# k2kobayashi/crank

Hardware: AMD Instinct MI355X
Metric: train frames/sec (higher is better)
Workload: dtype bf16; 1 GPU; vqvae trainer step (all sub-updates), VCC2020-shaped synthetic 80-dim mlfb, 64 utterances x 500 frames per GPU, 14 speakers; trainer=vqvae, global_batch=64, batch_len=500, parallelism=dp1

## Files before the change

### crank_amd/_lib.py

```python
import ctypes
import os
from .config import cfg
from ctypes import c_char_p, c_double, c_float, c_int, c_longlong, c_ulonglong, c_void_p

_HERE = os.path.dirname(os.path.abspath(__file__))
LIB_PATH = cfg.lib_path or os.path.join(_HERE, "libcrank_hip.so")
_lib = None

ERRORS = {1: "invalid argument", 2: "HIP runtime error", 3: "unsupported shape/configuration"}


class NetDesc(ctypes.Structure):
    _fields_ = [
        ("kind", c_int), ("in_ch", c_int), ("out_ch", c_int), ("kernel_size", c_int), ("layers", c_int),
        ("stacks", c_int), ("res_ch", c_int), ("gate_ch", c_int), ("skip_ch", c_int), ("aux_ch", c_int),
        ("conv_ch", c_int), ("causal", c_int), ("use_bias", c_int), ("slope", c_float), ("dropout", c_float),
    ]


COLLATE_MAX_STREAMS = 8


class CollateStream(ctypes.Structure):
    _fields_ = [("src", c_void_p), ("ld", c_int), ("col0", c_int), ("ncols", c_int), ("dst", c_void_p)]
# ... 8 lines not shown
    ]


P, I, LL, ULL, F, D = c_void_p, c_int, c_longlong, c_ulonglong, c_float, c_double

SIGNATURES = {
    "crk_net_create": (P, [ctypes.POINTER(NetDesc)]),
    "crk_net_destroy": (None, [P]),
    "crk_net_param_count": (LL, [P]),
    "crk_net_conv_count": (I, [P]),
    "crk_net_conv_info": (I, [P, I, ctypes.POINTER(c_longlong)]),
    "crk_net_saved_bytes": (LL, [P, I, I]),
    "crk_net_reserve": (I, [P, I, I]),
    "crk_net_scratch_bytes": (LL, [P, I, I]),
    "crk_debug_alloc_count": (LL, []),
    "crk_debug_net_paths": (I, [P, I, I]),
    "crk_seed_next": (I, [P, P, P]),
    "crk_nets_wnorm_bwd": (I, [I, P, P]),
    "crk_nets_prepare": (I, [I, P, P, ULL, P, P]),
    "crk_net_forward": (I, [P, P, ULL, P, I, P, I, P, I, P, I, I, I, ULL, P]),
    "crk_net_backward": (I, [P, P, ULL, P, P, I, P, I, P, I, P, I, F, P, I, P, I, I, I, ULL, P]),
    "crk_net_backward_scaled": (I, [P, P, ULL, P, P, I, P, I, P, I, P, I, F, P, I, P, I, I, I, ULL, P, P, P]),
    "crk_net_embed_grad_supported": (I, [P, I, I, I]),
    "crk_net_backward_embed": (I, [P, P, ULL, P, P, I, P, I, P, I, P, I, F, P, I, I, I, ULL, P, LL, I, I, I, P, P]),
    "crk_vq_forward": (I, [P, I, P, I, I, I, P, P, I, P, I, P]),
    "crk_vq_forward_fused": (I, [P, I, P, I, P, I, P, I, I, I, P, P, I, P, I, P, P, P, P, P]),
    "crk_vq_image_bytes": (LL, [I, I]),
    "crk_vq_image_build_multi": (I, [I, P, P, I, P, P]),
    "crk_vq_ema_scratch_bytes": (LL, [I, I, I]),
    "crk_vq_ema_stats": (I, [P, I, P, I, I, I, P, P, P, P]),
    "crk_vq_ema_apply": (I, [P, P, P, P, P, I, I, D, D, P]),
    "crk_vq_ema_partial": (I, [P, I, P, I, I, I, P, P]),
    "crk_vq_ema_reduce_multi": (I, [I, P, P, P, P, P, P, P]),
    "crk_vq_ema_apply_multi": (I, [I, P, P, P, P, P, P, P, D, D, P]),
    "crk_vq_ema_partial_multi": (I, [I, P, P, P, P, P, P, P, P]),
    "crk_vq_ema_reduce_size_multi": (I, [I, P, P, P, P, P, P, P, D, D, P]),
    "crk_vq_ema_blend_multi": (I, [I, P, P, P, P, P, P, D, P]),
    "crk_vq_ema_blend_image_multi": (I, [I, P, P, P, P, P, P, D, P, P]),
    "crk_stft_loss_multi_fwd": (I, [P, I, P, I, I, I, I, I, P, P, P, P, F, P, P, P]),
    "crk_stft_loss_multi_fwd_grad": (I, [P, I, P, I, I, I, I, I, P, P, P, P, F, P, P, I, P, P]),
    "crk_stft_loss_multi_bwd": (I, [P, I, P, I, I, I, I, I, P, P, P, P, F, P, P, I, P]),
    "crk_loss_scratch_floats": (I, []),
    "crk_masked_loss_fwd": (I, [P, I, P, I, F, P, LL, I, I, P, P, P]),
    "crk_masked_loss_bwd": (I, [P, I, P, I, F, P, LL, I, I, P, P, P, I, P, I, P]),
    "crk_masked_loss_both_fwd": (I, [P, I, P, I, P, LL, I, P, P, P]),
    "crk_weighted_sum": (I, [I, P, P, F, P, P]),
# ... 123 lines not shown
```

### crank_amd/config.py

```python
import contextlib
import os
import types

_get = os.environ.get


def _flag(name, default):
    v = _get(name)
    return default if v is None else v not in ("0", "")


def _read():
    return types.SimpleNamespace(
        precision=_get("CRANK_AMD_PRECISION", "bf16"),
        lib_path=_get("CRANK_AMD_LIB") or None,
        default_yaml=_get("CRANK_DEFAULT_YAML") or None,
        overlap_c=int(_get("CRANK_AMD_OVERLAP_C", "1") or 0),
        separate_ce=_flag("CRANK_AMD_SEPARATE_CE", False),
        separate_commit=_flag("CRANK_AMD_SEPARATE_COMMIT", False),
        recon_dense=_flag("CRANK_AMD_RECON_DENSE", False),
        stft_two_pass=_flag("CRANK_AMD_STFT_TWO_PASS", False),
        cond_sums=_flag("CRANK_AMD_COND_SUMS", True),
        force_dist=_flag("CRANK_AMD_FORCE_DIST", False),
        dist_backend=_get("CRANK_AMD_DIST_BACKEND") or None,
        dp_graph_collectives=_flag("CRANK_AMD_DP_GRAPH_COLLECTIVES", True),
        capture_mode=_get("CRANK_AMD_CAPTURE_MODE", "thread_local"),
        test_refuse_capture_rank=_get("CRANK_AMD_TEST_REFUSE_CAPTURE_RANK"),
    )


cfg = _read()


def reload():
    cfg.__dict__.update(_read().__dict__)


def torchrun():
    r = _get("RANK")
    return (None if r is None else int(r)), int(_get("LOCAL_RANK", "0")), int(_get("WORLD_SIZE", "1"))


@contextlib.contextmanager
def override(**kw):
    unknown = [k for k in kw if not hasattr(cfg, k)]
# ... 9 lines not shown
```

### crank_amd/csrc/conv_kernels.h

```cpp
#pragma once
#include <vector>

#include "common.h"
#include "switches.h"

#define CRK_TM 128

enum { MODE_PLAIN = 0, MODE_RESFWD = 1, MODE_BWDA = 2 };

struct ConvP {
  const float* xa; int lda; int cinA; float scaleA;
  const float* xb; int ldb; int cinB; float scaleB;
  int act_in; float slope;
  float drop_p; unsigned long long drop_seed;
  const unsigned long long* drop_seed_ptr;
  int cin, cin_pad;
  const float* xc; int ldc; int cinC; int cinC_pad;
  const uint16_t* w_hi; const uint16_t* w_lo;
  const uint16_t* wc_hi; const uint16_t* wc_lo;
  const uint16_t* w2_hi; const uint16_t* w2_lo;
  const float* bias; const float* bias2a; const float* bias2b;
  int cout, cout_pad, ktaps, dil, off0;
  int B, T, tiles_per_utt;
  float* y; int ldy; int accumulate; int act_out; float out_scale;
// ... 27 lines not shown

struct ConvEntry {
  int cout, cin, k;
  long long off_g, off_v, off_b;
  long long fw_off; int fw_rows, fw_kp, fw_row0;
  long long bw_off; int bw_rows, bw_kp, bw_col0;
  long long pt_off; int pt_rows, pt_row0, pt_cx, pt_taps, pt_tap0; float pt_scale;
  int pt_groups;
  long long pb_off;
  long long norm_off;
  long long fr_off; int fr_mode;
  long long bfr_off; int bfr_mode;
};

struct StackLayer {
  long long f_conv, f_aux, f_os;
  long long w_conv, w_aux, w_os;
  long long b_conv, b_out, b_skip;
  int dil, off0;
};
struct StackP {
  const float* x0;
  const float* c; int ldc; int aux_ch, aux_pad;
  float* saved;
  uint16_t *xb_hi, *xb_lo;
  uint16_t *zb_hi, *zb_lo;
  uint16_t *tb_hi, *tb_lo, *sg_hi, *sg_lo;
  uint16_t *cb_hi, *cb_lo;
  float* skip;
  const float* params;
  const uint16_t* whi; const uint16_t* wlo;
  const StackLayer* layers;
  int B, T, L, ktaps;
  int hl, hr, max_off;
  int tmo, tiles_per_utt;
  float drop_p; unsigned long long drop_seed; const unsigned long long* drop_seed_ptr;
  int o_xlo, o_zhi, o_zlo, o_chi, o_clo, o_whi, o_wlo, o_bias, o_tab, w_bytes, lds_bytes;
  int nw;
  int dbg;
  int ft, fh;
  int ft1;
  int o_zs, o_cs;
  int o_xf;
  const float* x_in; int ldx_in, in_ch, kp_first;
  long long f_first, b_first;
  long long f_h1, b_h1, f_h2, b_h2;
// ... 156 lines not shown
```

### crank_amd/csrc/net.hip

```cpp
#include <math.h>
#include <stdlib.h>
#include <string.h>

#include <deque>
#include <vector>

#include "conv_kernels.h"

struct crk_net_desc {
  int kind;
  int in_ch, out_ch, kernel_size, layers, stacks;
  int res_ch, gate_ch, skip_ch, aux_ch;
  int conv_ch;
  int causal;
  int use_bias;
  float slope;
  float dropout;
};

enum { ROLE_FIRST = 0, ROLE_CONV = 1, ROLE_AUX = 2, ROLE_OUT = 3, ROLE_SKIP = 4, ROLE_LAST1 = 5, ROLE_LAST2 = 6, ROLE_PLAIN = 7 };

struct ConvMeta {
  int role, layer, dilation;
};
// ... 620 lines not shown

static void tag_forward(Net* n, const float* saved, int B, int T, const Call& k, bool x3f) {
  if (!saved || !k.keep) return;
  const Net::FwdTag tag = {saved, B, T, k.mode, x3f};
  for (int i = 0; i < n->fwd_tag_count; i++)
    if (n->fwd_tags[i].saved == saved) { n->fwd_tags[i] = tag; return; }
  n->fwd_tags[n->fwd_tag_next] = tag;
  n->fwd_tag_next = (n->fwd_tag_next + 1) % 32;
  if (n->fwd_tag_count < 32) n->fwd_tag_count++;
}
static int check_forward_tag(const Net* n, const float* saved, int B, int T, int flags, int want, bool expects_x3f) {
  for (int i = 0; i < n->fwd_tag_count; i++) {
    const Net::FwdTag& t = n->fwd_tags[i];
    if (t.saved != saved) continue;
    if (t.B == B && t.T == T && t.mode == want && (want != 2 || t.x3f == expects_x3f)) return CRK_OK;
    fprintf(stderr, "[crank_hip] crk_net_backward: flags 0x%x (plane layout %d%s, B %d, T %d) do not match the forward that wrote this "
                    "workspace (layout %d%s, B %d, T %d): CRK_FLAG_PRECISE pairs with CRK_FLAG_PRECISE, CRK_FLAG_PRECISE | CRK_FLAG_BWD_PLAIN "
                    "with CRK_FLAG_FWD_PRECISE, plain with plain\n", flags, want, expects_x3f ? " x3f" : "", B, T, t.mode, t.x3f ? " x3f" : "", t.B, t.T);
    return CRK_ERR_ARG;
  }
  return CRK_OK;
}

struct FwdIo {
  const float* params; const float* x; int ldx; const float* c; int ldc; float* y; int ldy; float* saved; int B, T; hipStream_t s;
};
enum { FWD_CHAIN, FWD_CHAIN_LAYERS, FWD_FOLDED, FWD_FUSED, FWD_LAYERS };
static int fwd_form(const Net* n, const Route& rt, const Call& k, bool x3f, int* form) {
  if (n->d.kind == 2) { *form = rt.fused ? FWD_CHAIN : FWD_CHAIN_LAYERS; return CRK_OK; }
  const bool io16 = k.in16 && k.out16;
  if ((x3f || rt.gen_split) && !io16) {
    fprintf(stderr, "[crank_hip] crk_net_forward: x / y must be 16-byte aligned with row strides that are multiples of 4 floats\n");
    return CRK_ERR_ARG;
  }
  if (x3f || (rt.fold_fwd && io16)) *form = FWD_FOLDED;
  else if (rt.gen_split) return CRK_ERR_UNSUPPORTED;
  else *form = rt.fused ? FWD_FUSED : FWD_LAYERS;
  return CRK_OK;
}

static int fwd_chain(const Net* n, const Shape* r, const Call& k, const FwdIo& a) {
  if (!a.saved && k.keep) return CRK_ERR_ARG;
  const Route& rt = r->route[k.precise];
  const PsTables& Tb = r->ps;
  const long long N = (long long)a.B * a.T;
  PsP p = ps_base(n, a.B, a.T, a.params);
  p.x = a.x; p.ldx = a.ldx; p.cin = n->d.in_ch; p.y = a.y; p.ldy = a.ldy;
  if (k.keep) {
// ... 12 lines not shown
  const crk_net_desc& d = n->d;
  const int L = n->L;
  const long long N = (long long)a.B * a.T;
  if (L > 1 && !a.saved) return CRK_ERR_ARG;
  const float* in = a.x; int ldin = a.ldx;
  for (int i = 0; i < L; i++) {
    const ConvEntry& e = n->ents[n->idx_plain[i]];
    const int dil = n->meta[n->idx_plain[i]].dilation;
    const bool last = i == L - 1;
    ConvP p = conv_fw(n, a.B, a.T, e, a.params, in, ldin, last ? a.y : a.saved + (long long)i * N * d.conv_ch, last ? a.ldy : d.conv_ch);
    p.act_in = (i == 0) ? ACT_NONE : ACT_LRELU;
    p.ktaps = e.k; p.dil = dil; p.off0 = -((e.k - 1) / 2) * dil;
    RUN(conv_go(p, MODE_PLAIN, k.precise, a.s));
    in = p.y; ldin = p.ldy;
  }
  return CRK_OK;
}
static StackP stack_fwd_params(const Net* n, const Call& k, const FwdIo& a, bool lo) {
  const long long N = (long long)a.B * a.T;
  const GatedB16 gf = gated_b16(n, N);
  uint16_t* b16 = reinterpret_cast<uint16_t*>(a.saved + saved_f32_floats(n, N));
  StackP sp = stack_fwd_shape(n, a.B, a.T);
  sp.c = a.c; sp.ldc = a.ldc; sp.params = a.params;
  sp.skip = a.saved + gated_f32(n, N).skip;
  sp.whi = n->whi; sp.wlo = n->wlo; sp.layers = n->d_layers;
  if (!k.keep) return sp;
  sp.saved = a.saved;
  sp.xb_hi = b16 + gf.xb_hi; sp.zb_hi = b16 + gf.zb_hi; sp.tb_hi = b16 + gf.tb_hi; sp.sg_hi = b16 + gf.sg_hi;
  if (n->d.aux_ch > 0) sp.cb_hi = b16 + gf.cb_hi;
  if (!lo) { sp.fin_hi = b16 + gf.f_hi; sp.head_hi = b16 + gf.head_hi; return sp; }
  sp.xb_lo = b16 + gf.xb_lo; sp.zb_lo = b16 + gf.zb_lo; sp.tb_lo = b16 + gf.tb_lo; sp.sg_lo = b16 + gf.sg_lo;
  if (n->d.aux_ch > 0) sp.cb_lo = b16 + gf.cb_lo;
  return sp;
}
static int fwd_folded(const Net* n, const Route& rt, const Call& k, const FwdIo& a, bool x3f) {
  const crk_net_desc& d = n->d;
  const ConvEntry& ef = n->ents[n->idx_first];
  const ConvEntry& e1 = n->ents[n->idx_last1];
  const ConvEntry& e2 = n->ents[n->idx_last2];
  StackP sp = stack_fwd_params(n, k, a, false);
  sp.x_in = a.x; sp.ldx_in = a.ldx; sp.in_ch = d.in_ch; sp.kp_first = ef.fw_kp;
  sp.f_first = ef.fr_off; sp.b_first = ef.off_b;
  sp.f_h1 = e1.fr_off; sp.b_h1 = e1.off_b; sp.f_h2 = e2.fr_off; sp.b_h2 = e2.off_b;
  sp.y = a.y; sp.ldy = a.ldy; sp.out_ch = d.out_ch; sp.head_scale = (float)sqrt(1.0 / n->L);
  if (x3f || rt.gen_split) sp.ts_stride = ts_plane_stride((long long)a.B * a.T);
  if (x3f) { RUN(stack2x_fwd_plan(sp)); return launch_stack2x_fwd(sp, a.s); }
// ... 43 lines not shown
    const int dil = n->meta[n->idx_conv[l]].dilation;
    ConvP p = conv_fw(n, a.B, a.T, ec, a.params, X + l * P, 64, (l < L - 1) ? X + (l + 1) * P : nullptr, 64);
    p.ktaps = ec.k; p.dil = dil; p.off0 = fwd_off0(n, ec.k, dil);
    if (d.dropout > 0.f) { p.drop_p = d.dropout; p.drop_seed = layer_seed(k.seed_val, l); p.drop_seed_ptr = k.seed_ptr; }
    if (d.aux_ch > 0) {
      const ConvEntry& ea = n->ents[n->idx_aux[l]];
      p.xc = a.c; p.ldc = a.ldc; p.cinC = ea.cin; p.cinC_pad = ea.fw_kp;
      p.wc_hi = n->whi + ea.fw_off; p.wc_lo = n->wlo + ea.fw_off;
    }
    p.w2_hi = n->whi + eo.fw_off; p.w2_lo = n->wlo + eo.fw_off;
    p.bias2a = eo.off_b >= 0 ? a.params + eo.off_b : nullptr;
    p.bias2b = es.off_b >= 0 ? a.params + es.off_b : nullptr;
    p.skip = SKIP; p.skip_init = (l == 0);
    p.sv_ta = a.saved + lay.ta + l * P; p.sv_sb = a.saved + lay.sb + l * P; p.sv_z = a.saved + lay.z + l * P;
    RUN(conv_go(p, MODE_RESFWD, k.precise, a.s));
  }
  ConvP h1 = conv_fw(n, a.B, a.T, n->ents[n->idx_last1], a.params, SKIP, 64, H1, 64);
  h1.scaleA = (float)sqrt(1.0 / L); h1.act_in = head_act;
  RUN(conv_go(h1, MODE_PLAIN, k.precise, a.s));
  ConvP h2 = conv_fw(n, a.B, a.T, n->ents[n->idx_last2], a.params, H1, 64, a.y, a.ldy);
  h2.act_in = head_act;
  return conv_go(h2, MODE_PLAIN, k.precise, a.s);
}
extern "C" int crk_net_forward(void* h, const float* params, unsigned long long version, const float* x, int ldx,
                               const float* c, int ldc, float* y, int ldy, float* saved, int B, int T, int flags,
                               unsigned long long seed, void* stream) {
  Net* n = (Net*)h;
  if (!n || !params || !x || !y || B <= 0 || T <= 0) return CRK_ERR_ARG;
  const FwdIo a = {.params = params, .x = x, .ldx = ldx, .c = c, .ldc = ldc, .y = y, .ldy = ldy, .saved = saved, .B = B, .T = T,
                   .s = (hipStream_t)stream};
  const Call k = call_facts(flags, seed, true, x, ldx, y, ldy, nullptr, nullptr);
  const Shape* r = find_shape(n, B, T);
  if (!r) return not_reserved("crk_net_forward");
  const Route& rt = r->route[k.precise];
  const bool x3f = k.mode == 2 && r->route[0].x3f;
  RUN(ensure_prepared(n, params, version, a.s));
  tag_forward(n, saved, B, T, k, x3f);
  if (n->d.kind != 2 && (!saved || (n->d.aux_ch > 0 && !c))) return CRK_ERR_ARG;
  int form;
  RUN(fwd_form(n, rt, k, x3f, &form));
  switch (form) {
    case FWD_CHAIN: return fwd_chain(n, r, k, a);
    case FWD_CHAIN_LAYERS: return fwd_chain_layers(n, k, a);
    case FWD_FOLDED: return fwd_folded(n, rt, k, a, x3f);
    case FWD_FUSED: return fwd_fused(n, r, k, a);
  }
  return fwd_layers(n, k, a);
}

static int stack_cpg(const Net* n, int B, int T) {
  const int ncpu = (T + 63) / 64;
  const int groups = crk_sw().wg_groups;
  const int gsz = (B + groups - 1) / groups;
  int cpg = gsz * ncpu;
  if (crk_sw().wg_fill && n->d.kind != 2 && n->L > 0 && 256 / n->L > groups) {
    const int fill = 256 / n->L;
    const int c = (B * ncpu + fill - 1) / fill;
    if (c >= 1 && c < cpg) cpg = c;
  }
  return cpg < 1 ? 1 : cpg;
}
static int stack_groups(const Net* n, int B, int T) {
  const int total = B * ((T + 63) / 64), cpg = stack_cpg(n, B, T);
  return (total + cpg - 1) / cpg;
}

static int usum_nseg(const Net* n, int B, int T) {
  const int ncpu = (T + 63) / 64;
  return (stack_cpg(n, B, T) + 2 * ncpu - 2) / ncpu;
}
// ... 562 lines not shown
```

### crank_amd/csrc/stack2_kernels.hip

```cpp
#include "conv_kernels.h"

#include "stack_common.h"

#define S2_NCU 256
#define S2_PAIR_FACTOR 1.0

#if defined(S2_ABL) && (S2_ABL & 2)
#define mfma_bf16(a, b, c) s2_fake_mfma(a, b, c)
__device__ __forceinline__ f32x16 s2_fake_mfma(bf16x8 a, bf16x8 b, f32x16 c) {
  asm volatile("" ::"v"(a), "v"(b));
  return c;
}
#endif
#if defined(S2_ABL) && (S2_ABL & 4)
#define lds_frag(p) s2_fake_frag(p)
__device__ __forceinline__ bf16x8 s2_fake_frag(const unsigned char* p) {
  const unsigned v = (unsigned)(size_t)p;
  const sk_u32x4 q = {v, v, v, v};
  return __builtin_bit_cast(bf16x8, q);
}
#endif
#ifdef S2_PROF
__device__ unsigned long long s2_prof_buf[256 * 8 * 16];
__device__ unsigned long long s2_prof_res[1024 * 4];
// ... 62 lines not shown
  if (FOLD) {
    const __amdgpu_buffer_rsrc_t rxi = sk_rsrc(p.x_in, (long)p.B * p.T * p.ldx_in);
    int xrow = xr0, xcol = xc0;
#pragma unroll
    for (int u = 0; u < XQ; u++) {
      const int c4 = xcol * 4, t = t0 - p.hl + xrow;
      const bool on = xrow < R && t >= 0 && t < p.T && c4 < p.in_ch;
      xq[u] = __builtin_amdgcn_raw_buffer_load_b128(rxi, on ? (int)(((nbase + t) * p.ldx_in + c4) * 4) : SK_OOB, 0, 0);
      xrow += xdr; xcol += xdc;
      if (xcol >= ppr) { xcol -= ppr; xrow++; }
    }
    if (res_wave) {
      const int KF = p.kp_first >> 4;
#pragma unroll
      for (int kc = 0; kc < 8; kc++) awf[kc] = S2_WLOAD(p.f_first + (mt * KF + (kc < KF ? kc : 0)) * 512);
    }
#pragma unroll
    for (int q = 0; q < 4; q++)
      bfq[q] = (res_wave && p.b_first >= 0) ? *reinterpret_cast<const sk_f32x4*>(p.params + p.b_first + 32 * mt + 8 * q + 4 * half) : sk_f32x4{0.f, 0.f, 0.f, 0.f};
  }
  constexpr int CNQ = R * 16, CPER = AKC > 0 ? (CNQ + NT - 1) / NT : 1;
  float av[CPER][4];
  if (AKC > 0) {
#pragma unroll
    for (int it = 0; it < CPER; it++) {
      const int idx = tid + it * NT, r = idx >> 4, c4 = (idx & 15) << 2;
      const int tt = t0 - p.hl + r;
      const bool on = idx < CNQ && tt >= 0 && tt < p.T;
      const long n = nbase + tt;
#pragma unroll
      for (int j = 0; j < 4; j++) av[it][j] = (on && c4 + j < p.aux_ch) ? p.c[n * p.ldc + c4 + j] : 0.f;
    }
  }
  S2_T(12)
  constexpr int NBI = 16 * 256 / NT;
  float bv[NBI];
#pragma unroll
  for (int k = 0; k < NBI; k++) {
    const int i0 = __builtin_amdgcn_readfirstlane(tid + k * NT) & ~63;
    const int l = i0 >> 8, c0 = i0 & 255, c = c0 + lane;
    bv[k] = 0.f;
    if (l < p.L) {
      const long long bo = c0 < 128 ? p.layers[l].b_conv : (c0 < 192 ? p.layers[l].b_out : p.layers[l].b_skip);
      if (bo >= 0) bv[k] = p.params[bo + (c0 < 128 ? c : (c0 < 192 ? c - 128 : c - 192))] * ((c0 >= 128 && c0 < 192) ? 0.70710678118654752440f : 1.f);
    }
  }
  int tabv[2] = {0, 0};
#pragma unroll
  for (int u = 0; u < 2; u++)
    if (tid + u * NT < p.L * (int)(sizeof(StackLayer) / 4)) tabv[u] = reinterpret_cast<const int*>(p.layers)[tid + u * NT];
  static_assert(16 * sizeof(StackLayer) / 4 <= 2 * NT, "two table words per thread");

  constexpr int NWB = KT == 3 ? 3 : 4, NWB1 = KT == 3 ? 3 : 2;
  sk_u32x4 wa[NWB][4];
// ... 543 lines not shown
```

### crank_amd/net/module/vqvae2.py

```python
import torch

from ... import ops, parallel
from .flat import FlatModel
from .mlfb import LogMelFilterBankLayer
from .pwg import KIND_GENERATOR, MAX_CHANNELS, HipStack


class Quantizer:

    def __init__(self, owner, prefix, emb_dim, emb_size, decay=0.99, eps=1e-5, ema_flag=False, bdt_flag=False):
        self.owner, self.prefix = owner, prefix
        self.emb_dim, self.emb_size = emb_dim, emb_size
        self.decay, self.eps, self.ema_flag, self.bdt_flag = decay, eps, ema_flag, bdt_flag
        self.cb_offset = None
        self.training = True
        self.bucket, self.slot = None, 0
        self._img, self._img_epoch = None, -1

    def entries(self, base):
        self.cb_offset = base
        return [(self.prefix + "embedding.weight", base, (self.emb_size, self.emb_dim))]

    @property
    def n_params(self):
# ... 267 lines not shown
        if todo:
            ops.vq_image_build([q.weight for q in todo], [q._img for q in todo])
            for q in todo:
                q._img_epoch = self.codebook_epoch

    def train(self, mode=True):
        super().train(mode)
        for q in self.quantizers:
            q.training = mode
        return self

    @property
    def spkr_table(self):
        o = self.emb_offset
        return self.flat.data[o: o + self.spkr_size * self.emb_size].view(self.spkr_size, self.emb_size)

    def spkr_embedding(self, h):
        return ops.concat_embed(None, None, self.spkr_table, h, self, self.emb_offset, self.flat)

    def _get_dec_h(self, dec_h, spkrvec):
        a, b = dec_h if isinstance(dec_h, (tuple, list)) else (dec_h, None)
        if spkrvec is not None:
            if torch.is_grad_enabled() and ops.embed_owned_ok(self.decoders[0].net, a, b, spkrvec):
                return ops.concat_embed_owned(a, b, self.spkr_table, spkrvec, self, self.emb_offset)
            return ops.concat_embed(a, b, self.spkr_table, spkrvec, self, self.emb_offset, self.flat)
        return dec_h if b is None else torch.cat([a, b], dim=-1)

    def _pre(self, x):
        return self.preprocess_layer(x) if self.conf["use_raw"] else x

    def encode(self, x, enc_h=None):
        out = []
        cur = x
        dims = self.conf["emb_dim"][: self.conf["n_vq_stacks"]]
        ebuf = torch.empty(x.shape[0], x.shape[1], sum(dims), device=x.device, dtype=torch.float32)
        col = 0
        for n in range(self.conf["n_vq_stacks"]):
            cur = self.encoders[n](cur, c=enc_h if n == 0 else None, out=(ebuf, col))
            col += dims[n]
            out.append(cur)
        return out

    def decode(self, enc, dec_h, use_ema=True, detach=False, need_decoded=True, commit_mask=None, want_commit=False):
        dec = None
        emb_idxs, qxs, qidxs = [], [], []
        self._commits = []
        self.refresh_images()
# ... 95 lines not shown
```

### crank_amd/ops.py

```python
import ctypes

import torch

from . import _lib
from .config import cfg
from ._lib import check, ptr, stream_ptr

_PRECISION = cfg.precision


def set_precision(name):
    global _PRECISION
    if name not in ("bf16", "bf16x3", "bf16x3f"):
        raise ValueError(f"unknown precision {name!r} (bf16 | bf16x3 | bf16x3f)")
    _PRECISION = name


def get_precision():
    return _PRECISION


CRK_FLAG_PRECISE = 1
CRK_FLAG_NO_PARAM_GRAD = 2
CRK_FLAG_NO_SAVE = 4
CRK_FLAG_DEFER_WNORM = 8
CRK_FLAG_SEED_ON_DEVICE = 16
CRK_FLAG_FWD_PRECISE = 32
CRK_FLAG_BWD_PLAIN = 64


def _flags(skip_param_grads=False, no_save=False, precision=None, defer_wnorm=False, backward=False):
    prec = precision or _PRECISION
    if prec == "bf16x3f":
        pbits = CRK_FLAG_FWD_PRECISE if backward else (CRK_FLAG_PRECISE | CRK_FLAG_BWD_PLAIN)
    else:
        pbits = CRK_FLAG_PRECISE if prec == "bf16x3" else 0
    return (pbits | (CRK_FLAG_NO_PARAM_GRAD if skip_param_grads else 0) | (CRK_FLAG_NO_SAVE if no_save else 0)
            | (CRK_FLAG_DEFER_WNORM if defer_wnorm else 0))


class _ScalarArena:

    def __init__(self, device, n=256):
        self.buf = torch.empty(n, device=device, dtype=torch.float32)
        self.pos = 0


_ARENA = None


def begin_scalar_arena(device):
# ... 60 lines not shown
        self.seed_state.fill_(v)

    def next_seed(self):
        out = torch.empty(1, dtype=torch.int64, device=self.seed_state.device)
        check(_lib.lib().crk_seed_next(ptr(self.seed_state), ptr(out), stream_ptr()), "crk_seed_next")
        return out

    def saved_bytes(self, B, T):
        key = (B, T, _PRECISION)
        v = self._saved_bytes.get(key)
        if v is None:
            check(_lib.lib().crk_net_reserve(self.handle, B, T), "crk_net_reserve")
            v = self._saved_bytes[key] = _lib.lib().crk_net_saved_bytes(self.handle, B, T)
        return v

    def embed_grad_supported(self, B, T):
        key = ("embed", B, T, _PRECISION)
        v = self._saved_bytes.get(key)
        if v is None:
            self.saved_bytes(B, T)
            v = self._saved_bytes[key] = bool(_lib.lib().crk_net_embed_grad_supported(self.handle, B, T, _flags(backward=True)))
        return v

    def __del__(self):
        try:
            if getattr(self, "handle", None):
                _lib.lib().crk_net_destroy(self.handle)
                self.handle = None
        except Exception:
            pass


class _NetFn(torch.autograd.Function):

    @staticmethod
    def forward(ctx, x, c, flat, net, owner, offset, dx_scale, no_save=False, ybuf=None, ycol=0, emb=None):
        L = _lib.lib()
        B, T = x.shape[0], x.shape[1]
        if emb is not None and not (c is not None and emb.run == T and net.embed_grad_supported(B, T)):
            raise RuntimeError("conditioning built by concat_embed_owned fed to a net that cannot own its table gradient")
        xk, ldx = _rows(x)
        ck, ldc = (None, 0) if c is None else _rows(c)
        if ybuf is None:
            y = torch.empty(B, T, net.out_ch, device=x.device, dtype=torch.float32)
        else:
            y = ybuf[..., ycol: ycol + net.out_ch]
        ldy = y.stride(1)
        nbytes = net.saved_bytes(B, T)
        saved = torch.empty(max(nbytes // 4, 1), device=x.device, dtype=torch.float32)
        seed_t = net.next_seed() if net.dropout > 0 else None
        params = flat.data_ptr() + 4 * offset
        check(
            L.crk_net_forward(net.handle, params, owner.version, ptr(xk), ldx, ptr(ck), ldc, ptr(y), ldy,
                              ptr(saved), B, T, _flags(no_save=no_save) | (CRK_FLAG_SEED_ON_DEVICE if seed_t is not None else 0), ptr(seed_t),
                              stream_ptr()),
            "crk_net_forward",
        )
        ctx.net, ctx.owner, ctx.offset, ctx.dx_scale, ctx.seed = net, owner, offset, dx_scale, seed_t
        ctx.precision = _PRECISION
        ctx.ld = (ldx, ldc)
        ctx.version = owner.version
        ctx.save_for_backward(xk, ck if ck is not None else torch.empty(0, device=x.device), flat)
        ctx.saved_ws = saved
        ctx.has_c = c is not None
        ctx.emb = emb
        return y

    @staticmethod
    def backward(ctx, dy):
        L = _lib.lib()
        net, owner = ctx.net, ctx.owner
        xk, ck, flat = ctx.saved_tensors
        if not ctx.has_c:
            ck = None
        ldx, ldc = ctx.ld
        B, T = xk.shape[0], xk.shape[1]
        dyk, lddy = _rows(dy)
        dx = torch.empty(B, T, net.in_ch, device=dy.device, dtype=torch.float32) if ctx.needs_input_grad[0] else None
        dc = None
        if ctx.has_c and ctx.needs_input_grad[1]:
# ... 90 lines not shown
        return dx, None, None, None, None, None, None, None, None


def net_ce(net, owner, offset, x, target, dx_scale=1.0, ignore_index=-100):
    if net.dropout > 0:
        raise ValueError("net_ce: nets with dropout go through net_apply + cross_entropy")
    return _NetCEFn.apply(x, owner.flat, net, owner, offset, dx_scale, target, ignore_index, not torch.is_grad_enabled())


def nets_wnorm_bwd(nets):
    arr = (ctypes.c_void_p * len(nets))(*[n.handle for n in nets])
    check(_lib.lib().crk_nets_wnorm_bwd(len(nets), arr, stream_ptr()), "crk_nets_wnorm_bwd")


def nets_prepare(nets, param_ptrs, version, bump_step=None):
    arr = (ctypes.c_void_p * len(nets))(*[n.handle for n in nets])
    par = (ctypes.c_void_p * len(nets))(*param_ptrs)
    check(_lib.lib().crk_nets_prepare(len(nets), arr, par, version, ptr(bump_step), stream_ptr()), "crk_nets_prepare")


def net_apply(net, owner, offset, x, c=None, dx_scale=1.0, out=None):
    ybuf, ycol = out if out is not None else (None, 0)
    emb = getattr(c, "_crk_embed", None) if c is not None else None
    return _NetFn.apply(x, c, owner.flat, net, owner, offset, dx_scale, not torch.is_grad_enabled(), ybuf, ycol, emb)


class _AliasCatFn(torch.autograd.Function):

    @staticmethod
    def forward(ctx, *xs):
        B, T = xs[0].shape[0], xs[0].shape[1]
        W = sum(x.shape[2] for x in xs)
        ctx.widths = [x.shape[2] for x in xs]
        return xs[0].as_strided((B, T, W), (T * W, W, 1))

    @staticmethod
    def backward(ctx, d):
        out, off = [], 0
        for w in ctx.widths:
            out.append(d[..., off: off + w])
            off += w
        return tuple(out)


def cat_channels(xs):
    xs = list(xs)
# ... 638 lines not shown

    @staticmethod
    def backward(ctx, dout):
        L = _lib.lib()
        (ik,) = ctx.saved_tensors
        ca, cb, E, rows, run, N = ctx.geom
        dk, ld = _rows(dout)
        if ctx.owner is not None and not ctx.owner.skip_param_grads:
            ctx.owner.grads_clean = False
            g = ctx.owner.grad_flat[ctx.tab_offset: ctx.tab_offset + rows * E]
            scratch = torch.empty(L.crk_embed_bwd_scratch_floats(N, E, rows), device=dk.device, dtype=torch.float32)
            check(L.crk_embed_bwd_run(ptr(dk), ld, ca + cb, E, ptr(ik), run, N, rows, ptr(g), ptr(scratch), stream_ptr()),
                  "crk_embed_bwd_run")
        da = dk[..., :ca] if (ca and ctx.needs_input_grad[0]) else None
        db = dk[..., ca:ca + cb] if (cb and ctx.needs_input_grad[1]) else None
        return da, db, None, None, None, None, None


def concat_embed(a, b, table, idx, owner=None, tab_offset=0, flat=None):
    return _ConcatEmbedFn.apply(a, b, table, idx, owner, tab_offset, flat)


class EmbedCond:
    __slots__ = ("idx", "run", "c0", "E", "rows", "owner", "tab_offset")


def embed_owned_ok(net, a, b, idx):
    if not cfg.cond_sums or idx.dim() != 2:
        return False
    if (a is not None and a.requires_grad) or (b is not None and b.requires_grad):
        return False
    B, T = idx.shape
    return _label_runs(idx)[1] == T and net.embed_grad_supported(B, T)


def concat_embed_owned(a, b, table, idx, owner, tab_offset):
    with torch.no_grad():
        out, ik, run, (ca, cb, E) = _concat_embed_fwd(a, b, table, idx)
    e = EmbedCond()
    e.idx, e.run, e.c0, e.E, e.rows, e.owner, e.tab_offset = ik, run, ca + cb, E, table.shape[0], owner, tab_offset
    out._crk_embed = e
    return out


def adam_step(flat, grad, exp_avg, exp_avg_sq, lr_dev, step_dev, beta1=0.9, beta2=0.999, eps=1e-8, clear_grads=False,
              defer_bump=False):
    check(_lib.lib().crk_adam_step(ptr(flat), ptr(grad), ptr(exp_avg), ptr(exp_avg_sq), flat.numel(), ptr(lr_dev),
                                   ptr(step_dev), beta1, beta2, eps, (1 if clear_grads else 0) | (2 if defer_bump else 0),
                                   stream_ptr()), "crk_adam_step")


def radam_step(flat, grad, exp_avg, exp_avg_sq, lr_dev, step_dev, beta1=0.9, beta2=0.999, eps=1e-8, clear_grads=False,
               defer_bump=False):
    check(_lib.lib().crk_radam_step(ptr(flat), ptr(grad), ptr(exp_avg), ptr(exp_avg_sq), flat.numel(), ptr(lr_dev),
                                    ptr(step_dev), beta1, beta2, eps, (1 if clear_grads else 0) | (2 if defer_bump else 0),
                                    stream_ptr()), "crk_radam_step")


def lamb_tile():
    return int(_lib.lib().crk_lamb_tile())


# ... 21 lines not shown
```

### include/crank_hip.h

```cpp
#ifndef CRANK_HIP_H
#define CRANK_HIP_H
#ifdef __cplusplus
extern "C" {
#endif

#define CRK_OK 0
#define CRK_ERR_ARG 1
#define CRK_ERR_HIP 2
#define CRK_ERR_UNSUPPORTED 3

#define CRK_FLAG_PRECISE 1
#define CRK_FLAG_NO_PARAM_GRAD 2
#define CRK_FLAG_NO_SAVE 4
#define CRK_FLAG_DEFER_WNORM 8

#define CRK_FLAG_SEED_ON_DEVICE 16
#define CRK_FLAG_FWD_PRECISE 32
#define CRK_FLAG_BWD_PLAIN 64

typedef struct crk_net_desc {
  int kind;
  int in_ch, out_ch, kernel_size, layers, stacks;
  int res_ch, gate_ch, skip_ch, aux_ch;
  int conv_ch;
// ... 7 lines not shown
void crk_net_destroy(void* net);
long long crk_net_param_count(void* net);
int crk_net_conv_count(void* net);
int crk_net_conv_info(void* net, int i, long long* out9);
long long crk_net_saved_bytes(void* net, int B, int T);
int crk_net_reserve(void* net, int B, int T);
long long crk_net_scratch_bytes(void* net, int B, int T);
int crk_net_forward(void* net, const float* params, unsigned long long version, const float* x, int ldx,
                    const float* c, int ldc, float* y, int ldy, float* saved, int B, int T, int flags,
                    unsigned long long seed, void* stream);
int crk_net_backward(void* net, const float* params, unsigned long long version, float* grads, const float* x,
                     int ldx, const float* c, int ldc, const float* dy, int lddy, float* dx, int lddx, float dx_scale,
                     float* dc, int lddc, const float* saved, int B, int T, int flags, unsigned long long seed,
                     void* stream);
int crk_net_backward_scaled(void* net, const float* params, unsigned long long version, float* grads, const float* x,
                            int ldx, const float* c, int ldc, const float* dy, int lddy, float* dx, int lddx, float dx_scale,
                            float* dc, int lddc, const float* saved, int B, int T, int flags, unsigned long long seed,
                            const float* dy_num, const float* dy_den, void* stream);
int crk_net_embed_grad_supported(void* net, int B, int T, int flags);
int crk_net_backward_embed(void* net, const float* params, unsigned long long version, float* grads, const float* x, int ldx,
                           const float* c, int ldc, const float* dy, int lddy, float* dx, int lddx, float dx_scale,
                           const float* saved, int B, int T, int flags, unsigned long long seed, const long long* idx,
                           long long run, int c0, int E, int n_rows, float* dtable, void* stream);

int crk_seed_next(unsigned long long* state, unsigned long long* out, void* stream);

int crk_nets_wnorm_bwd(int n_nets, void* const* nets, void* stream);
int crk_nets_prepare(int n_nets, void* const* nets, const float* const* params, unsigned long long version,
                     float* bump_step, void* stream);

int crk_vq_forward(const float* x, int ldx, const float* codebook, int N, int D, int K, long long* idx, float* e,
                   int lde, float* qx, int ldq, void* stream);
int crk_vq_forward_fused(const float* x, int ldx, const float* add, int ldadd, float* xsum, int ldsum, const float* codebook,
                         int N, int D, int K, long long* idx, float* e, int lde, float* qx, int ldq,
                         const unsigned char* mask, float* commit_out2, float* scratch, const void* image, void* stream);
long long crk_vq_image_bytes(int K, int D);
int crk_vq_image_build_multi(int nq, const float* const* codebooks, const int* K, int D, void* const* images, void* stream);
long long crk_vq_ema_scratch_bytes(int N, int D, int K);
int crk_vq_ema_stats(const float* x, int ldx, const long long* idx, int N, int D, int K, int* counts, long long* sums,
                     void* scratch, void* stream);
int crk_vq_ema_apply(const int* counts, const long long* sums, float* ema_size, float* ema_w, float* codebook, int D,
                     int K, double decay, double eps, void* stream);
int crk_vq_ema_partial(const float* x, int ldx, const long long* idx, int N, int D, int K, void* scratch, void* stream);
int crk_vq_ema_reduce_multi(int nq, const void* const* scratch, const int* N, const int* D, const int* K,
                            int* const* counts, long long* const* sums, void* stream);
int crk_vq_ema_apply_multi(int nq, const int* const* counts, const long long* const* sums, float* const* ema_size,
// ... 228 lines not shown
```

Before: 22.06 million frames/s.

## Gather speaker-embedding conditioning lazily inside decoder stack forward kernel

Instead of materialising the concatenated decoder conditioning tensor (encoder outputs plus speaker embedding rows), the join is deferred. The decoder's fused stack kernel reads the aux channels directly from the two source buffers and the embedding table by speaker index. This removes one concat kernel and a full-size intermediate write and read per step. It adds branching to the aux load path, a meta-device placeholder tensor, and a fallback that materialises the tensor when the route is unsupported or another net consumes it.

```diff
diff --git a/crank_amd/_lib.py b/crank_amd/_lib.py
--- a/crank_amd/_lib.py
+++ b/crank_amd/_lib.py
@@ -54,6 +54,8 @@
     "crk_net_backward": (I, [P, P, ULL, P, P, I, P, I, P, I, P, I, F, P, I, P, I, I, I, ULL, P]),
     "crk_net_backward_scaled": (I, [P, P, ULL, P, P, I, P, I, P, I, P, I, F, P, I, P, I, I, I, ULL, P, P, P]),
     "crk_net_embed_grad_supported": (I, [P, I, I, I]),
+    "crk_net_embed_fwd_supported": (I, [P, I, I, I]),
+    "crk_net_forward_embed": (I, [P, P, ULL, P, I, P, I, I, P, I, I, P, I, P, LL, P, I, P, I, I, I, ULL, P]),
     "crk_net_backward_embed": (I, [P, P, ULL, P, P, I, P, I, P, I, P, I, F, P, I, I, I, ULL, P, LL, I, I, I, P, P]),
     "crk_vq_forward": (I, [P, I, P, I, I, I, P, P, I, P, I, P]),
     "crk_vq_forward_fused": (I, [P, I, P, I, P, I, P, I, I, I, P, P, I, P, I, P, P, P, P, P]),
diff --git a/crank_amd/config.py b/crank_amd/config.py
--- a/crank_amd/config.py
+++ b/crank_amd/config.py
@@ -21,6 +21,7 @@
         recon_dense=_flag("CRANK_AMD_RECON_DENSE", False),
         stft_two_pass=_flag("CRANK_AMD_STFT_TWO_PASS", False),
         cond_sums=_flag("CRANK_AMD_COND_SUMS", True),
+        lazy_join=_flag("CRANK_AMD_LAZY_JOIN", True),
         force_dist=_flag("CRANK_AMD_FORCE_DIST", False),
         dist_backend=_get("CRANK_AMD_DIST_BACKEND") or None,
         dp_graph_collectives=_flag("CRANK_AMD_DP_GRAPH_COLLECTIVES", True),
diff --git a/crank_amd/csrc/conv_kernels.h b/crank_amd/csrc/conv_kernels.h
--- a/crank_amd/csrc/conv_kernels.h
+++ b/crank_amd/csrc/conv_kernels.h
@@ -73,6 +73,8 @@
 struct StackP {
   const float* x0;
   const float* c; int ldc; int aux_ch, aux_pad;
+  const float* c2; int ldc2; int c_ca, c_cb;
+  const float* c_tab; const long long* c_idx;
   float* saved;
   uint16_t *xb_hi, *xb_lo;
   uint16_t *zb_hi, *zb_lo;
diff --git a/crank_amd/csrc/net.hip b/crank_amd/csrc/net.hip
--- a/crank_amd/csrc/net.hip
+++ b/crank_amd/csrc/net.hip
@@ -666,8 +666,10 @@
   return CRK_OK;
 }
 
+struct CondGather { const float* b; int ldb, ca, cb; const float* table; const long long* idx; };
 struct FwdIo {
   const float* params; const float* x; int ldx; const float* c; int ldc; float* y; int ldy; float* saved; int B, T; hipStream_t s;
+  const CondGather* cg;
 };
 enum { FWD_CHAIN, FWD_CHAIN_LAYERS, FWD_FOLDED, FWD_FUSED, FWD_LAYERS };
 static int fwd_form(const Net* n, const Route& rt, const Call& k, bool x3f, int* form) {
@@ -726,6 +728,7 @@
   uint16_t* b16 = reinterpret_cast<uint16_t*>(a.saved + saved_f32_floats(n, N));
   StackP sp = stack_fwd_shape(n, a.B, a.T);
   sp.c = a.c; sp.ldc = a.ldc; sp.params = a.params;
+  if (a.cg) { sp.c2 = a.cg->b; sp.ldc2 = a.cg->ldb; sp.c_ca = a.cg->ca; sp.c_cb = a.cg->cb; sp.c_tab = a.cg->table; sp.c_idx = a.cg->idx; }
   sp.skip = a.saved + gated_f32(n, N).skip;
   sp.whi = n->whi; sp.wlo = n->wlo; sp.layers = n->d_layers;
   if (!k.keep) return sp;
@@ -815,22 +818,23 @@
   h2.act_in = head_act;
   return conv_go(h2, MODE_PLAIN, k.precise, a.s);
 }
-extern "C" int crk_net_forward(void* h, const float* params, unsigned long long version, const float* x, int ldx,
-                               const float* c, int ldc, float* y, int ldy, float* saved, int B, int T, int flags,
-                               unsigned long long seed, void* stream) {
+static int net_forward_impl(void* h, unsigned long long version, int flags, unsigned long long seed, const FwdIo& a) {
   Net* n = (Net*)h;
+  const float *params = a.params, *x = a.x, *c = a.c; float *y = a.y, *saved = a.saved;
+  const int B = a.B, T = a.T, ldx = a.ldx, ldy = a.ldy;
   if (!n || !params || !x || !y || B <= 0 || T <= 0) return CRK_ERR_ARG;
-  const FwdIo a = {.params = params, .x = x, .ldx = ldx, .c = c, .ldc = ldc, .y = y, .ldy = ldy, .saved = saved, .B = B, .T = T,
-                   .s = (hipStream_t)stream};
   const Call k = call_facts(flags, seed, true, x, ldx, y, ldy, nullptr, nullptr);
   const Shape* r = find_shape(n, B, T);
   if (!r) return not_reserved("crk_net_forward");
   const Route& rt = r->route[k.precise];
   const bool x3f = k.mode == 2 && r->route[0].x3f;
+  int form;
+  if (a.cg) {
+    if (n->d.kind == 2 || x3f || !(rt.fold_fwd && k.in16 && k.out16)) return CRK_ERR_UNSUPPORTED;
+  }
   RUN(ensure_prepared(n, params, version, a.s));
   tag_forward(n, saved, B, T, k, x3f);
   if (n->d.kind != 2 && (!saved || (n->d.aux_ch > 0 && !c))) return CRK_ERR_ARG;
-  int form;
   RUN(fwd_form(n, rt, k, x3f, &form));
   switch (form) {
     case FWD_CHAIN: return fwd_chain(n, r, k, a);
@@ -839,6 +843,32 @@
     case FWD_FUSED: return fwd_fused(n, r, k, a);
   }
   return fwd_layers(n, k, a);
+}
+extern "C" int crk_net_forward(void* h, const float* params, unsigned long long version, const float* x, int ldx,
+                               const float* c, int ldc, float* y, int ldy, float* saved, int B, int T, int flags,
+                               unsigned long long seed, void* stream) {
+  const FwdIo a = {.params = params, .x = x, .ldx = ldx, .c = c, .ldc = ldc, .y = y, .ldy = ldy, .saved = saved, .B = B, .T = T,
+                   .s = (hipStream_t)stream, .cg = nullptr};
+  return net_forward_impl(h, version, flags, seed, a);
+}
+extern "C" int crk_net_embed_fwd_supported(void* h, int B, int T, int flags) {
+  Net* n = (Net*)h;
+  if (!n || B <= 0 || T <= 0 || n->d.kind == 2 || n->d.aux_ch <= 0 || (flags & CRK_FLAG_PRECISE)) return 0;
+  return route_at(n, B, T, false).fold_fwd ? 1 : 0;
+}
+extern "C" int crk_net_forward_embed(void* h, const float* params, unsigned long long version, const float* x, int ldx,
+                                     const float* a, int lda, int ca, const float* b, int ldb, int cb, const float* table,
+                                     int E, const long long* idx, long long run, float* y, int ldy, float* saved, int B, int T,
+                                     int flags, unsigned long long seed, void* stream) {
+  Net* n = (Net*)h;
+  if (!n || !table || !idx || run != T || ca < 0 || cb < 0 || E < 1 || (ca > 0 && !a) || (cb > 0 && !b) ||
+      ca + cb + E != n->d.aux_ch)
+    return CRK_ERR_ARG;
+  if (flags & CRK_FLAG_PRECISE) return CRK_ERR_UNSUPPORTED;
+  const CondGather cg = {b, ldb, ca, cb, table, idx};
+  const FwdIo io = {.params = params, .x = x, .ldx = ldx, .c = ca > 0 ? a : table, .ldc = lda, .y = y, .ldy = ldy, .saved = saved,
+                    .B = B, .T = T, .s = (hipStream_t)stream, .cg = &cg};
+  return net_forward_impl(h, version, flags, seed, io);
 }
 
 static int stack_cpg(const Net* n, int B, int T) {
diff --git a/crank_amd/csrc/stack2_kernels.hip b/crank_amd/csrc/stack2_kernels.hip
--- a/crank_amd/csrc/stack2_kernels.hip
+++ b/crank_amd/csrc/stack2_kernels.hip
@@ -108,6 +108,8 @@
   constexpr int CNQ = R * 16, CPER = AKC > 0 ? (CNQ + NT - 1) / NT : 1;
   float av[CPER][4];
   if (AKC > 0) {
+    const int ca = p.c_tab ? p.c_ca : p.aux_ch, cab = p.c_tab ? p.c_ca + p.c_cb : p.aux_ch;
+    const float* trow = p.c_tab ? p.c_tab + p.c_idx[nbase] * (long)(p.aux_ch - cab) - cab : p.c;
 #pragma unroll
     for (int it = 0; it < CPER; it++) {
       const int idx = tid + it * NT, r = idx >> 4, c4 = (idx & 15) << 2;
@@ -115,7 +117,11 @@
       const bool on = idx < CNQ && tt >= 0 && tt < p.T;
       const long n = nbase + tt;
 #pragma unroll
-      for (int j = 0; j < 4; j++) av[it][j] = (on && c4 + j < p.aux_ch) ? p.c[n * p.ldc + c4 + j] : 0.f;
+      for (int j = 0; j < 4; j++) {
+        const int col = c4 + j;
+        const float* src = col < ca ? p.c + n * p.ldc + col : (col < cab ? p.c2 + n * p.ldc2 + (col - ca) : trow + col);
+        av[it][j] = (on && col < p.aux_ch) ? *src : 0.f;
+      }
     }
   }
   S2_T(12)
diff --git a/crank_amd/net/module/vqvae2.py b/crank_amd/net/module/vqvae2.py
--- a/crank_amd/net/module/vqvae2.py
+++ b/crank_amd/net/module/vqvae2.py
@@ -313,7 +313,8 @@
         a, b = dec_h if isinstance(dec_h, (tuple, list)) else (dec_h, None)
         if spkrvec is not None:
             if torch.is_grad_enabled() and ops.embed_owned_ok(self.decoders[0].net, a, b, spkrvec):
-                return ops.concat_embed_owned(a, b, self.spkr_table, spkrvec, self, self.emb_offset)
+                return ops.concat_embed_owned(a, b, self.spkr_table, spkrvec, self, self.emb_offset,
+                                              consumer=self.decoders[0].net)
             return ops.concat_embed(a, b, self.spkr_table, spkrvec, self, self.emb_offset, self.flat)
         return dec_h if b is None else torch.cat([a, b], dim=-1)
 
diff --git a/crank_amd/ops.py b/crank_amd/ops.py
--- a/crank_amd/ops.py
+++ b/crank_amd/ops.py
@@ -27,6 +27,7 @@
 CRK_FLAG_SEED_ON_DEVICE = 16
 CRK_FLAG_FWD_PRECISE = 32
 CRK_FLAG_BWD_PLAIN = 64
+CRK_ERR_UNSUPPORTED = 3
 
 
 def _flags(skip_param_grads=False, no_save=False, precision=None, defer_wnorm=False, backward=False):
@@ -133,6 +134,14 @@
             v = self._saved_bytes[key] = bool(_lib.lib().crk_net_embed_grad_supported(self.handle, B, T, _flags(backward=True)))
         return v
 
+    def embed_fwd_supported(self, B, T):
+        key = ("embed_fwd", B, T, _PRECISION)
+        v = self._saved_bytes.get(key)
+        if v is None:
+            self.saved_bytes(B, T)
+            v = self._saved_bytes[key] = bool(_lib.lib().crk_net_embed_fwd_supported(self.handle, B, T, _flags()))
+        return v
+
     def __del__(self):
         try:
             if getattr(self, "handle", None):
@@ -151,7 +160,9 @@
         if emb is not None and not (c is not None and emb.run == T and net.embed_grad_supported(B, T)):
             raise RuntimeError("conditioning built by concat_embed_owned fed to a net that cannot own its table gradient")
         xk, ldx = _rows(x)
-        ck, ldc = (None, 0) if c is None else _rows(c)
+        lazy = emb is not None and emb.lazy is not None
+        assert not lazy or emb.consumer is net, "a deferred conditioning reached a net it was not paired with"
+        ck, ldc = (None, 0) if (c is None or lazy) else _rows(c)
         if ybuf is None:
             y = torch.empty(B, T, net.out_ch, device=x.device, dtype=torch.float32)
         else:
@@ -161,12 +172,23 @@
         saved = torch.empty(max(nbytes // 4, 1), device=x.device, dtype=torch.float32)
         seed_t = net.next_seed() if net.dropout > 0 else None
         params = flat.data_ptr() + 4 * offset
-        check(
-            L.crk_net_forward(net.handle, params, owner.version, ptr(xk), ldx, ptr(ck), ldc, ptr(y), ldy,
-                              ptr(saved), B, T, _flags(no_save=no_save) | (CRK_FLAG_SEED_ON_DEVICE if seed_t is not None else 0), ptr(seed_t),
-                              stream_ptr()),
-            "crk_net_forward",
-        )
+        fl = _flags(no_save=no_save) | (CRK_FLAG_SEED_ON_DEVICE if seed_t is not None else 0)
+        if lazy:
+            ak, lda, ca, bk, ldb, cb, table = emb.lazy
+            rc = L.crk_net_forward_embed(net.handle, params, owner.version, ptr(xk), ldx, ptr(ak), lda, ca, ptr(bk), ldb, cb,
+                                         ptr(table), emb.E, ptr(emb.idx), emb.run, ptr(y), ldy, ptr(saved), B, T, fl,
+                                         ptr(seed_t), stream_ptr())
+            if rc == CRK_ERR_UNSUPPORTED:
+                ck, ldc = _rows(_embed_materialise(emb))
+                lazy = False
+            else:
+                check(rc, "crk_net_forward_embed")
+        if not lazy:
+            check(
+                L.crk_net_forward(net.handle, params, owner.version, ptr(xk), ldx, ptr(ck), ldc, ptr(y), ldy,
+                                  ptr(saved), B, T, fl, ptr(seed_t), stream_ptr()),
+                "crk_net_forward",
+            )
         ctx.net, ctx.owner, ctx.offset, ctx.dx_scale, ctx.seed = net, owner, offset, dx_scale, seed_t
         ctx.precision = _PRECISION
         ctx.ld = (ldx, ldc)
@@ -303,6 +325,13 @@
 def net_apply(net, owner, offset, x, c=None, dx_scale=1.0, out=None):
     ybuf, ycol = out if out is not None else (None, 0)
     emb = getattr(c, "_crk_embed", None) if c is not None else None
+    if emb is not None and emb.lazy is not None and emb.consumer is not net:
+        c = _embed_materialise(emb)
+        done = EmbedCond()
+        for k in EmbedCond.__slots__:
+            setattr(done, k, getattr(emb, k))
+        done.lazy = done.consumer = None
+        emb = c._crk_embed = done
     return _NetFn.apply(x, c, owner.flat, net, owner, offset, dx_scale, not torch.is_grad_enabled(), ybuf, ycol, emb)
 
 
@@ -987,7 +1016,7 @@
 
 
 class EmbedCond:
-    __slots__ = ("idx", "run", "c0", "E", "rows", "owner", "tab_offset")
+    __slots__ = ("idx", "run", "c0", "E", "rows", "owner", "tab_offset", "lazy", "consumer", "shape")
 
 
 def embed_owned_ok(net, a, b, idx):
@@ -999,10 +1028,29 @@
     return _label_runs(idx)[1] == T and net.embed_grad_supported(B, T)
 
 
-def concat_embed_owned(a, b, table, idx, owner, tab_offset):
-    with torch.no_grad():
-        out, ik, run, (ca, cb, E) = _concat_embed_fwd(a, b, table, idx)
+def _embed_materialise(e):
+    ak, lda, ca, bk, ldb, cb, table = e.lazy
+    B, T, C = e.shape
+    out = torch.empty(B, T, C, device=table.device, dtype=torch.float32)
+    check(_lib.lib().crk_concat_embed_run(ptr(ak), lda, ca, ptr(bk), ldb, cb, ptr(table), e.E, ptr(e.idx), e.run, B * T,
+                                          ptr(out), C, stream_ptr()), "crk_concat_embed_run")
+    return out
+
+
+def concat_embed_owned(a, b, table, idx, owner, tab_offset, consumer=None):
     e = EmbedCond()
+    B, T = idx.shape
+    if cfg.lazy_join and consumer is not None and consumer.embed_fwd_supported(B, T):
+        ak, lda = (None, 0) if a is None else _rows(a)
+        bk, ldb = (None, 0) if b is None else _rows(b)
+        ca, cb, E = (0 if a is None else a.shape[-1]), (0 if b is None else b.shape[-1]), table.shape[1]
+        ik, run = _label_runs(idx)
+        e.lazy, e.consumer, e.shape = (ak, lda, ca, bk, ldb, cb, table), consumer, (B, T, ca + cb + E)
+        out = torch.empty(B, T, ca + cb + E, device="meta", dtype=torch.float32)
+    else:
+        with torch.no_grad():
+            out, ik, run, (ca, cb, E) = _concat_embed_fwd(a, b, table, idx)
+        e.lazy, e.consumer, e.shape = None, None, tuple(out.shape)
     e.idx, e.run, e.c0, e.E, e.rows, e.owner, e.tab_offset = ik, run, ca + cb, E, table.shape[0], owner, tab_offset
     out._crk_embed = e
     return out
diff --git a/include/crank_hip.h b/include/crank_hip.h
--- a/include/crank_hip.h
+++ b/include/crank_hip.h
@@ -53,6 +53,12 @@
                            const float* c, int ldc, const float* dy, int lddy, float* dx, int lddx, float dx_scale,
                            const float* saved, int B, int T, int flags, unsigned long long seed, const long long* idx,
                            long long run, int c0, int E, int n_rows, float* dtable, void* stream);
+
+int crk_net_embed_fwd_supported(void* net, int B, int T, int flags);
+int crk_net_forward_embed(void* net, const float* params, unsigned long long version, const float* x, int ldx, const float* a,
+                          int lda, int ca, const float* b, int ldb, int cb, const float* table, int E, const long long* idx,
+                          long long run, float* y, int ldy, float* saved, int B, int T, int flags, unsigned long long seed,
+                          void* stream);
 
 int crk_seed_next(unsigned long long* state, unsigned long long* out, void* stream);
 
```

Measured after the change: 22.25 million frames/s (median of 6 runs). Within noise of the previous version (+0.8%).
